# knowles-group/iterative-solver

Measured on AMD Instinct MI355X. Metric: subspace-update GB/s (gemm_inner+axpy) at N=1e8, 8 roots; 1/2/4/8 GPU, higher is better.
Workload: dtype f64

## Files before the change

iterative-solver_amd/csrc/context.hip:

```cpp
#include <immintrin.h>

#include <unistd.h>

#include <algorithm>
#include <atomic>
#include <chrono>
#include <condition_variable>
#include <cstdio>
#include <cstdlib>
#include <cstring>
#include <memory>
#include <mutex>
#include <thread>

#include "ssp_internal.h"

namespace {
thread_local std::string g_last_error;

size_t round_block(size_t bytes) {
  if (bytes < (size_t(1) << 20)) return (bytes + 255) & ~size_t(255);
  const size_t g = size_t(2) << 20;
  return (bytes + g - 1) / g * g;
}
// ... 380 lines not shown

int ssp_ledger_entry(ssp_ctx* ctx, int i, const char** name, long long* calls, double* kernel_ms, double* bytes) {
  SSP_CHECK_CTX(ctx);
  SSP_TRY(ssp::ledger_resolve(ctx));
  if (i < 0 || size_t(i) >= ctx->ledger.size()) return ssp::set_error(SSP_ERR_ARG, "ssp_ledger_entry: bad index");
  const auto& e = ctx->ledger[i];
  if (name) *name = e.name.c_str();
  if (calls) *calls = e.calls;
  if (kernel_ms) *kernel_ms = e.ms;
  if (bytes) *bytes = e.bytes;
  return SSP_OK;
}

const char* ssp_last_error(void) { return g_last_error.c_str(); }

const char* ssp_version(void) { return "subspace_hip 0.1 (gfx950, fp64)"; }

int ssp_device_count(void) {
  int n = 0;
  if (hipGetDeviceCount(&n) != hipSuccess) return 0;
  return n;
}

int ssp_ctx_create(int device, ssp_ctx** out) {
  if (!out) return ssp::set_error(SSP_ERR_ARG, "ssp_ctx_create: null out");
  *out = nullptr;
  int ndev = 0;
  SSP_TRY_HIP(hipGetDeviceCount(&ndev));
  if (device < 0 || device >= ndev)
    return ssp::set_error(SSP_ERR_ARG, "ssp_ctx_create: device " + std::to_string(device) + " not present");
  SSP_TRY_HIP(hipSetDevice(device));
  auto* ctx = new ssp_ctx();
  ctx->device = device;
  hipDeviceProp_t prop;
  if (hipGetDeviceProperties(&prop, device) == hipSuccess && prop.multiProcessorCount > 0)
    ctx->num_cus = prop.multiProcessorCount;
  if (const char* rs = std::getenv("SSP_ROW_SHAPE")) ctx->row_stride = std::string(rs) == "stride";
  if (const char* pc = std::getenv("SSP_PUBLISH")) ctx->publish_copy = std::string(pc) == "copy";
  if (const char* ex = std::getenv("SSP_EXACT_MAX")) ctx->exact_max = size_t(std::strtoull(ex, nullptr, 10));
  if (const char* ip = std::getenv("SSP_INNER_PER_CU")) ctx->inner_per_cu = std::max(1, std::atoi(ip));
  if (const char* op = std::getenv("SSP_OUTER_WG_PER_CU")) ctx->outer_per_cu = std::max(1, std::atoi(op));
  if (const char* fp = std::getenv("SSP_FUSED_PER_CU")) ctx->fused_per_cu = std::max(1, std::atoi(fp));
  if (const char* tw = std::getenv("SSP_TRANSFORM_WIDE")) ctx->transform_wide = std::atoi(tw) != 0;
  if (const char* sm = std::getenv("SSP_SELECT_MERGE")) ctx->select_rank = std::string(sm) != "tree";
  if (const char* lt = std::getenv("SSP_LEDGER_TIMING")) ctx->ledger_dispatch = std::string(lt) == "dispatch";
  ctx->ledger_detail = std::getenv("SSP_LEDGER_DETAIL") != nullptr;
  if (const char* ss = std::getenv("SSP_SYNTH_SHAPE")) {
    ctx->synth_stride = std::string(ss) == "stride";
    ctx->synth_window = std::string(ss) == "window";
  }
  if (const char* sm = std::getenv("SSP_SYNTH_MERGE")) ctx->synth_merge = std::atoi(sm) != 0;
  if (const char* df = std::getenv("SSP_DEFER_FILL")) ctx->defer_fill = std::atoi(df) != 0;
  if (const char* dout = std::getenv("SSP_DEFER_OUTER")) ctx->defer_outer = std::atoi(dout) != 0;
  if (const char* ct = std::getenv("SSP_COMM_TIMEOUT_S")) {
    const double v = std::atof(ct);
    if (v > 0) ctx->comm_timeout_s = v;
  }
  if (hipStreamCreateWithFlags(&ctx->stream, hipStreamNonBlocking) != hipSuccess) {
    delete ctx;
    return ssp::set_error(SSP_ERR_HIP, "hipStreamCreate failed");
  }
  int s = ssp::ensure_partial(ctx, size_t(1) << 20);
  if (s == SSP_OK) s = ssp::ensure_result(ctx, size_t(1) << 16);
  if (s == SSP_OK) {
    const size_t bytes = sizeof(unsigned) * ssp::kFoldLine * (ssp::kFoldShards + 1);
    if (hipMalloc(reinterpret_cast<void**>(&ctx->fold_counter), bytes) != hipSuccess ||
        hipMemsetAsync(ctx->fold_counter, 0, bytes, ctx->stream) != hipSuccess)
      s = ssp::set_error(SSP_ERR_NOMEM, "allocation of the reduction counter failed");
  }
  if (s != SSP_OK) {
    ssp_ctx_destroy(ctx);
    return s;
  }
  *out = ctx;
  return SSP_OK;
}

int ssp_ctx_destroy(ssp_ctx* ctx) {
  if (!ctx) return SSP_OK;
  (void)hipSetDevice(ctx->device);
  ctx->pending_fills.clear();
  ctx->pending_outer.discard();
  (void)ssp::p2p_detach(ctx);
  if (ctx->stream) (void)hipStreamSynchronize(ctx->stream);
  if (ctx->comm) ncclCommDestroy(ctx->comm);
  if (ctx->dev_err_host) (void)hipHostFree(ctx->dev_err_host);
  for (auto& e : ctx->ledger)
    for (auto& pr : e.pending) {
      (void)hipEventDestroy(pr.first);
      (void)hipEventDestroy(pr.second);
    }
  for (auto ev : ctx->event_pool) (void)hipEventDestroy(ev);
  for (auto& b : ctx->free_blocks) (void)hipFree(b.second);
  for (auto& b : ctx->live_blocks) (void)hipFree(b.first);
  if (ctx->partial) (void)hipFree(ctx->partial);
  if (ctx->result_dev) (void)hipFree(ctx->result_dev);
  if (ctx->result_host) (void)hipHostFree(ctx->result_host);
  if (ctx->pub_flag) (void)hipHostFree(ctx->pub_flag);
  if (ctx->fold_counter) (void)hipFree(ctx->fold_counter);
  if (ctx->async_dev) (void)hipFree(ctx->async_dev);
  if (ctx->async_host) (void)hipHostFree(ctx->async_host);
  if (ctx->async_flag) (void)hipHostFree(ctx->async_flag);
  if (ctx->synth_mask) (void)hipFree(ctx->synth_mask);
  if (ctx->ring_dev) (void)hipFree(ctx->ring_dev);
  if (ctx->ring_host) (void)hipHostFree(ctx->ring_host);
  for (auto& r : ctx->retired_rings) {
    if (r.first) (void)hipFree(r.first);
    if (r.second) (void)hipHostFree(r.second);
  }
  if (ctx->stream) (void)hipStreamDestroy(ctx->stream);
  delete ctx;
  return SSP_OK;
}

void* ssp_ctx_stream(ssp_ctx* ctx) {
  if (!ctx) return nullptr;
  (void)ssp::enter(ctx);
  return reinterpret_cast<void*>(ctx->stream);
}

int ssp_synchronize(ssp_ctx* ctx) {
  SSP_CHECK_CTX(ctx);
  return ssp::sync_stream(ctx, "synchronize");
}

int ssp_alloc(ssp_ctx* ctx, size_t n, double** out) {
  SSP_CHECK_CTX(ctx);
  if (!out) return ssp::set_error(SSP_ERR_ARG, "ssp_alloc: null out");
  const size_t bytes = round_block(std::max<size_t>(n, 1) * sizeof(double));
  auto it = ctx->free_blocks.find(bytes);
  void* p = nullptr;
  if (it != ctx->free_blocks.end()) {
    p = it->second;
    ctx->free_blocks.erase(it);
    ctx->bytes_cached -= bytes;
  } else {
    hipError_t e = hipMalloc(&p, bytes);
    if (e != hipSuccess) {
      (void)hipGetLastError();
      (void)hipStreamSynchronize(ctx->stream);
      for (auto& b : ctx->free_blocks) (void)hipFree(b.second);
      ctx->free_blocks.clear();
      ctx->bytes_cached = 0;
      if (hipMalloc(&p, bytes) != hipSuccess) {
        (void)hipGetLastError();
        return ssp::set_error(SSP_ERR_NOMEM, "ssp_alloc: out of HBM for " + std::to_string(bytes) + " bytes");
      }
    }
// ... 208 lines not shown
```

iterative-solver_amd/csrc/kernels_panel.hip:

```cpp
#include <algorithm>
#include <cstdio>
#include <cstddef>
#include <cstdlib>
#include <vector>

#include "ssp_internal.h"

namespace {

using ssp::kBlock;

__device__ __forceinline__ double2 ld2(const double* p) { return *reinterpret_cast<const double2*>(p); }
template <bool SC>
__device__ __forceinline__ double2 sc2(double2 v, double s) {
  return SC ? make_double2(v.x * s, v.y * s) : v;
}
template <bool SC>
__device__ __forceinline__ double sc1(double v, double s) {
  return SC ? v * s : v;
}

struct InnerArgs {
  const double* x[ssp::kInnerRows];
  const double* y[ssp::kInnerCols];
// ... 222 lines not shown
        }
#pragma unroll
        for (int j = 0; j < K; ++j)
#pragma unroll
          for (int u = 0; u < U; ++u) {
            acc[j][u & 1] = fma(xv[u].x, yv[j][u].x, acc[j][u & 1]);
            acc[j][u & 1] = fma(xv[u].y, yv[j][u].y, acc[j][u & 1]);
          }
      },
      [&](size_t p) {
        const double2 xv = sc2<SC>(ld2(a.x[0] + 2 * p), xs);
#pragma unroll
        for (int j = 0; j < K; ++j) {
          const double2 yv = sc2<SC>(ld2(a.y[j] + 2 * p), ys[j]);
          acc[j][0] = fma(xv.x, yv.x, acc[j][0]);
          acc[j][0] = fma(xv.y, yv.y, acc[j][0]);
        }
      },
      [&](size_t e) {
#pragma unroll
        for (int j = 0; j < K; ++j) acc[j][0] = fma(sc1<SC>(a.x[0][e], xs), sc1<SC>(a.y[j][e], ys[j]), acc[j][0]);
      });
  __shared__ double red[kBlock / 64][K];
  const int lane = threadIdx.x & 63, wave = threadIdx.x >> 6;
#pragma unroll
  for (int j = 0; j < K; ++j) {
    double v = acc[j][0] + acc[j][1];
#pragma unroll
    for (int off = 32; off > 0; off >>= 1) v += __shfl_down(v, off, 64);
    if (lane == 0) red[wave][j] = v;
  }
  __syncthreads();
  if (int(threadIdx.x) < K) {
    double v = red[0][threadIdx.x];
#pragma unroll
    for (int w = 1; w < kBlock / 64; ++w) v += red[w][threadIdx.x];
    ssp::store_partial(a.partial + size_t(blockIdx.x) * K + threadIdx.x, v);
  }
  if (a.tail.counter) ssp::fold_tail<K>(a.partial, a.tail);
}

struct OuterArgs {
  const double* x[ssp::kOuterSrc];
  double* y[ssp::kOuterDst];
  int k;
  int m;
  int set;
  int epi_mask;
  size_t n;
  const double* alpha_dev;
  const double* scale_dev;
  double alpha[ssp::kOuterAlpha];
  double epi[ssp::kOuterDst];
};
static_assert(sizeof(OuterArgs) <= 4000, "kernel argument block too large");
static_assert(ssp::PendingOuter::kSrc == ssp::kOuterSrc && ssp::PendingOuter::kDst == ssp::kOuterDst,
              "pending_outer.h records one launch");

constexpr int kOuterWin = 4;

template <int M, bool DEV, bool SET, bool SC = false, bool EPI = false>
__global__ __launch_bounds__(kBlock) void k_gemm_outer(const OuterArgs a) {
  static_assert(!EPI || (SET && !SC), "the epilogue rides on the unscaled write-only form");
  using ssp::ld2nt;
  using ssp::st2nt;
  using cdouble = const __attribute__((address_space(4))) double;
  const auto alpha = [&](int idx) { return DEV ? ((cdouble*)a.alpha_dev)[idx] : a.alpha[idx]; };
  const auto scale = [&](int idx) { return SC ? ((cdouble*)a.scale_dev)[idx] : 1.0; };
  constexpr int U = M > 8 ? 2 : kOuterWin;
  const int lane = threadIdx.x & 63;
  const size_t gw = size_t(blockIdx.x) * (kBlock / 64) + (threadIdx.x >> 6);
  const size_t nw = size_t(gridDim.x) * (kBlock / 64);
  const size_t n2 = a.n >> 1, win = 64 * U;
  const double2 z2 = make_double2(0, 0);
  for (size_t c = gw; c * win < n2; c += nw) {
    const size_t p0 = c * win + lane;
    bool ok[U];
#pragma unroll
    for (int u = 0; u < U; ++u) ok[u] = p0 + 64 * u < n2;
    double2 acc[U][M];
#pragma unroll
    for (int u = 0; u < U; ++u)
#pragma unroll
      for (int j = 0; j < M; ++j) acc[u][j] = (j < a.m && ok[u] && !SET) ? ld2nt(a.y[j] + 2 * (p0 + 64 * u)) : z2;
    if constexpr (SC && !SET) {
#pragma unroll
      for (int u = 0; u < U; ++u)
#pragma unroll
        for (int j = 0; j < M; ++j)
          if (j < a.m) acc[u][j] = sc2<SC>(acc[u][j], scale(a.k + j));
    }
    int i = 0;
    for (; i + 4 <= a.k; i += 4) {
      double2 xv[4][U];
#pragma unroll
      for (int b = 0; b < 4; ++b)
#pragma unroll
        for (int u = 0; u < U; ++u) xv[b][u] = ok[u] ? ld2nt(a.x[i + b] + 2 * (p0 + 64 * u)) : z2;
      if constexpr (SC) {
#pragma unroll
        for (int b = 0; b < 4; ++b)
#pragma unroll
          for (int u = 0; u < U; ++u) xv[b][u] = sc2<SC>(xv[b][u], scale(i + b));
      }
#pragma unroll
      for (int b = 0; b < 4; ++b)
#pragma unroll
        for (int j = 0; j < M; ++j) {
          if (j < a.m) {
            const double al = alpha((i + b) * a.m + j);
#pragma unroll
            for (int u = 0; u < U; ++u) {
              acc[u][j].x = fma(al, xv[b][u].x, acc[u][j].x);
              acc[u][j].y = fma(al, xv[b][u].y, acc[u][j].y);
            }
          }
        }
    }
    for (; i < a.k; ++i) {
      double2 xv[U];
#pragma unroll
      for (int u = 0; u < U; ++u) xv[u] = ok[u] ? ld2nt(a.x[i] + 2 * (p0 + 64 * u)) : z2;
      if constexpr (SC) {
#pragma unroll
        for (int u = 0; u < U; ++u) xv[u] = sc2<SC>(xv[u], scale(i));
      }
#pragma unroll
      for (int j = 0; j < M; ++j) {
        if (j < a.m) {
          const double al = alpha(i * a.m + j);
#pragma unroll
          for (int u = 0; u < U; ++u) {
            acc[u][j].x = fma(al, xv[u].x, acc[u][j].x);
            acc[u][j].y = fma(al, xv[u].y, acc[u][j].y);
          }
        }
      }
    }
    if constexpr (EPI) {
      constexpr int B = M == 8 ? 2 : 1;
#pragma unroll
      for (int j0 = 0; j0 < M; j0 += B) {
        double2 ev[B][U];
        bool on[B];
#pragma unroll
        for (int b = 0; b < B; ++b) {
          on[b] = j0 + b < a.m && ((a.epi_mask >> (j0 + b)) & 1);
          if (on[b]) {
#pragma unroll
            for (int u = 0; u < U; ++u) ev[b][u] = ok[u] ? ld2nt(a.x[a.k + j0 + b] + 2 * (p0 + 64 * u)) : z2;
          }
        }
#pragma unroll
        for (int b = 0; b < B; ++b) {
          if (on[b]) {
            const double ea = a.epi[j0 + b];
#pragma unroll
            for (int u = 0; u < U; ++u) {
              acc[u][j0 + b].x = fma(ea, ev[b][u].x, acc[u][j0 + b].x);
              acc[u][j0 + b].y = fma(ea, ev[b][u].y, acc[u][j0 + b].y);
            }
          }
        }
      }
    }
#pragma unroll
    for (int u = 0; u < U; ++u)
      if (ok[u])
#pragma unroll
        for (int j = 0; j < M; ++j)
          if (j < a.m) st2nt(a.y[j] + 2 * (p0 + 64 * u), acc[u][j]);
  }
  if ((a.n & 1) && blockIdx.x == 0 && threadIdx.x < a.m) {
    const size_t e = a.n - 1;
    const int j = threadIdx.x;
    double v = SET ? 0.0 : sc1<SC>(a.y[j][e], scale(a.k + j));
    for (int i = 0; i < a.k; ++i) v = fma(alpha(i * a.m + j), sc1<SC>(a.x[i][e], scale(i)), v);
    if constexpr (EPI) {
      if ((a.epi_mask >> j) & 1) v = fma(a.epi[j], a.x[a.k + j][e], v);
    }
    a.y[j][e] = v;
  }
}

struct AxpyInnerArgs {
  const double* x;
  const double* z;
  double* y[ssp::kOuterDst];
  double c[ssp::kOuterDst];
  int m;
  size_t n;
  double* partial;
  ssp::FoldTail tail;
};

constexpr int kFusedU = 4;

template <int M>
__global__ __launch_bounds__(kBlock) void k_axpy_inner(const AxpyInnerArgs a) {
  using ssp::ld2nt;
  using ssp::st2nt;
  double acc[M];
#pragma unroll
  for (int j = 0; j < M; ++j) acc[j] = 0;
  ssp::for_windows<kFusedU>(
      a.n,
      [&](size_t p0) {
        double2 xv[kFusedU], zv[kFusedU];
#pragma unroll
        for (int u = 0; u < kFusedU; ++u) xv[u] = ld2nt(a.x + 2 * (p0 + 64 * u));
#pragma unroll
        for (int u = 0; u < kFusedU; ++u) zv[u] = ld2nt(a.z + 2 * (p0 + 64 * u));
#pragma unroll
        for (int j = 0; j < M; ++j) {
          if (j < a.m) {
            double2 y[kFusedU];
#pragma unroll
            for (int u = 0; u < kFusedU; ++u) y[u] = ld2nt(a.y[j] + 2 * (p0 + 64 * u));
#pragma unroll
            for (int u = 0; u < kFusedU; ++u) {
              y[u].x = fma(a.c[j], xv[u].x, y[u].x);
              y[u].y = fma(a.c[j], xv[u].y, y[u].y);
              st2nt(a.y[j] + 2 * (p0 + 64 * u), y[u]);
              acc[j] = fma(y[u].x, zv[u].x, acc[j]);
// ... 672 lines not shown
template <bool SC>
int launch_inner_sym_t(ssp_ctx* ctx, const InnerArgs& a, unsigned grid) {
  switch ((a.m + 3) / 4) {
    case 1: launch_inner_sym_g<1, SC>(ctx, a, grid); break;
    case 2: launch_inner_sym_g<2, SC>(ctx, a, grid); break;
    case 3: launch_inner_sym_g<3, SC>(ctx, a, grid); break;
    default: launch_inner_sym_g<4, SC>(ctx, a, grid); break;
  }
  SSP_TRY_HIP(hipGetLastError());
  return SSP_OK;
}

int launch_inner_sym(ssp_ctx* ctx, const InnerArgs& a, unsigned grid, bool sc) {
  return sc ? launch_inner_sym_t<true>(ctx, a, grid) : launch_inner_sym_t<false>(ctx, a, grid);
}

template <bool SC>
int launch_inner_sc(ssp_ctx* ctx, const InnerArgs& a, unsigned grid, bool pre) {
  const int mg = (a.m + 3) / 4, need = (a.k + 3) / 4;
  switch (mg) {
    case 1: return launch_inner_mg<1, SC>(ctx, grid, a, need, pre);
    case 2: return launch_inner_mg<2, SC>(ctx, grid, a, need, pre);
    case 3: return launch_inner_mg<3, SC>(ctx, grid, a, need, false);
    default: return launch_inner_mg<4, SC>(ctx, grid, a, need, false);
  }
}

int launch_inner(ssp_ctx* ctx, const InnerArgs& a, unsigned grid, bool sc, bool pre = false) {
  return sc ? launch_inner_sc<true>(ctx, a, grid, pre) : launch_inner_sc<false>(ctx, a, grid, pre);
}

template <bool DEV, bool SET, bool SC, bool EPI = false>
void launch_outer_t(ssp_ctx* ctx, unsigned grid, const OuterArgs& a) {
  if (a.m <= 1)
    SSP_LAUNCH((k_gemm_outer<1, DEV, SET, SC, EPI>), dim3(grid), dim3(kBlock), 0, ctx->stream, a);
  else if (a.m <= 2)
    SSP_LAUNCH((k_gemm_outer<2, DEV, SET, SC, EPI>), dim3(grid), dim3(kBlock), 0, ctx->stream, a);
  else if (a.m <= 4)
    SSP_LAUNCH((k_gemm_outer<4, DEV, SET, SC, EPI>), dim3(grid), dim3(kBlock), 0, ctx->stream, a);
  else if (a.m <= 8)
    SSP_LAUNCH((k_gemm_outer<8, DEV, SET, SC, EPI>), dim3(grid), dim3(kBlock), 0, ctx->stream, a);
  else
    SSP_LAUNCH((k_gemm_outer<16, DEV, SET, SC, EPI>), dim3(grid), dim3(kBlock), 0, ctx->stream, a);
}

template <bool SC>
void launch_outer_sc(ssp_ctx* ctx, unsigned grid, const OuterArgs& a) {
  if (a.alpha_dev)
    a.set ? launch_outer_t<true, true, SC>(ctx, grid, a) : launch_outer_t<true, false, SC>(ctx, grid, a);
  else
    a.set ? launch_outer_t<false, true, SC>(ctx, grid, a) : launch_outer_t<false, false, SC>(ctx, grid, a);
}

int launch_outer(ssp_ctx* ctx, const OuterArgs& a) {
  const unsigned grid = ssp::stream_grid(ctx, a.n / 2 + 1, kOuterWin, unsigned(ctx->outer_per_cu));
  if (a.epi_mask) {
    if (!a.set || a.scale_dev || a.k + a.m > ssp::kOuterSrc)
      return ssp::set_error(SSP_ERR_ARG, "gemm_outer: epilogue terms on a launch that cannot carry them");
    a.alpha_dev ? launch_outer_t<true, true, false, true>(ctx, grid, a)
                : launch_outer_t<false, true, false, true>(ctx, grid, a);
    SSP_TRY_HIP(hipGetLastError());
    return SSP_OK;
  }
  a.scale_dev ? launch_outer_sc<true>(ctx, grid, a) : launch_outer_sc<false>(ctx, grid, a);
  SSP_TRY_HIP(hipGetLastError());
  return SSP_OK;
}

int ng_inst(int need) { return need <= 4 ? need : need <= 6 ? 6 : need <= 8 ? 8 : need <= 12 ? 12 : 16; }
std::string shape_tag(const char* kind, int a, int b, int c, int d, bool sc) {
  char t[96];
  std::snprintf(t, sizeof(t), "%s<%d,%d> %dx%d%s", kind, a, b, c, d, sc ? " sc" : "");
  return t;
}

bool any_scaled(const double* s, int n) {
  for (int i = 0; s && i < n; ++i)
    if (s[i] != 1.0) return true;
  return false;
}

}

extern "C" {

int ssp_gemm_inner(ssp_ctx* ctx, const double* const* xx, int m, const double* const* yy, int k, size_t n,
                   double* out) {
  return ssp_gemm_inner_scaled(ctx, xx, nullptr, m, yy, nullptr, k, n, out);
}

int ssp_gemm_inner_scaled(ssp_ctx* ctx, const double* const* xx, const double* xs, int m, const double* const* yy,
                          const double* ys, int k, size_t n, double* out) {
  SSP_CHECK_CTX(ctx);
  if (m < 0 || k < 0) return ssp::set_error(SSP_ERR_ARG, "ssp_gemm_inner: negative dimension");
  if (m * k > 0 && !out) return ssp::set_error(SSP_ERR_ARG, "ssp_gemm_inner: null out");
  if (m == 0 || k == 0) return SSP_OK;
  SSP_TRY(check_ptrs(xx, m, n, "ssp_gemm_inner"));
  SSP_TRY(check_ptrs(yy, k, n, "ssp_gemm_inner"));
  const bool swap = m > k;
  const double* const* rows = swap ? yy : xx;
  const double* const* cols = swap ? xx : yy;
  const int R = swap ? k : m, C = swap ? m : k;
  std::vector<double> rs(size_t(R), 1.0), cs(size_t(C), 1.0);
  for (int i = 0; i < m; ++i) (swap ? cs : rs)[size_t(i)] = xs ? xs[i] : 1.0;
  for (int j = 0; j < k; ++j) (swap ? rs : cs)[size_t(j)] = ys ? ys[j] : 1.0;
  const bool sc = any_scaled(rs.data(), R) || any_scaled(cs.data(), C);
  int pad = -1;
// ... 85 lines not shown
        const int cols_per_launch = 4 * ng_max((mr + 3) / 4);
        for (int c0 = 0; c0 < C2; c0 += cols_per_launch) {
          InnerArgs a{};
          a.m = mr;
          a.k = std::min(cols_per_launch, C2 - c0);
          a.n = n;
          for (int i = 0; i < a.m; ++i) {
            a.x[i] = rows[r0 + i];
            a.xs[i] = rs[size_t(r0 + i)];
          }
          for (int j = 0; j < a.k; ++j) {
            a.y[j] = cols[c0 + j];
            a.ys[j] = cs[size_t(c0 + j)];
          }
          const bool sc_launch = any_scaled(a.xs, a.m) || any_scaled(a.ys, a.k);
          const unsigned grid = inner_grid(ctx, n);
          SSP_TRY(ssp::ensure_partial(ctx, size_t(grid) * a.m * a.k));
          a.partial = ctx->partial;
          const bool pre = pad >= 0 && c0 == 0;
          if (r0 == 0 && c0 == 0)
            ls.detail(shape_tag(pre ? "mfma-pre" : "mfma", (a.m + 3) / 4, ng_inst((a.k + 3) / 4), a.m, a.k, sc_launch));
          SSP_TRY(launch_inner(ctx, a, grid, sc_launch, pre));
          const bool last = r0 + ssp::kInnerRows >= R && c0 + cols_per_launch >= C2;
          SSP_TRY(ssp::launch_reduce_partials(ctx, ctx->partial, int(grid), a.m, a.k, ctx->result_dev, C2, r0, c0, &tail,
                                              last));
        }
      }
    }
  }
  std::vector<double> t(swap || pad >= 0 ? total : 0);
  double* dst = swap || pad >= 0 ? t.data() : out;
  if (tail.counter) {
    SSP_TRY(ssp::fold_finish(ctx, tail, dst));
  } else {
    SSP_TRY(ssp::reduce_fetch(ctx, dst, total));
  }
  if (pad >= 0) {
    for (int i = 0; i < R; ++i)
      for (int j = 0; j < C; ++j) t[size_t(i) * C + j] = t[size_t(i) * C2 + (j < R ? j : j + pad)];
    if (!swap) {
      std::copy(t.begin(), t.begin() + long(size_t(R) * C), out);
      return SSP_OK;
    }
  }
  if (!swap) return SSP_OK;
  for (int i = 0; i < m; ++i)
    for (int j = 0; j < k; ++j) out[size_t(i) * k + j] = t[size_t(j) * m + i];
  return SSP_OK;
}

}

namespace {
int launch_record(ssp_ctx* ctx, const ssp::PendingOuter::Record& r) {
  const int e = r.terms();
  ssp::LedgerScope ls(ctx, r.set ? "gemm_outer_set" : "gemm_outer", 8.0 * r.n * (r.k + r.m + e));
  OuterArgs a{};
  a.k = r.k;
  a.m = r.m;
  a.set = 1;
  a.n = r.n;
  for (int i = 0; i < r.k; ++i) a.x[i] = r.x[i];
  for (int j = 0; j < r.m; ++j) a.y[j] = r.y[j];
  if (e > 0) {
    a.epi_mask = int(r.mask);
    for (int j = 0; j < r.m; ++j) {
      const bool on = (r.mask >> j) & 1u;
      a.x[r.k + j] = on ? r.ex[j] : nullptr;
      a.epi[j] = on ? r.ea[j] : 0.0;
    }
  }
  const bool dev = r.k * r.m > ssp::kOuterAlpha;
  if (dev) {
    void* p;
    SSP_TRY(ssp::upload_small(ctx, r.alpha, size_t(r.k) * r.m * sizeof(double), &p));
    a.alpha_dev = static_cast<const double*>(p);
    SSP_TRY(ssp::flush_uploads(ctx));
  } else {
    std::copy(r.alpha, r.alpha + r.k * r.m, a.alpha);
  }
  const int mi = a.m <= 1 ? 1 : a.m <= 2 ? 2 : a.m <= 4 ? 4 : a.m <= 8 ? 8 : 16;
  std::string tag = shape_tag(dev ? "dev" : "arg", mi, a.set, a.k, a.m, false);
  if (e > 0) tag += " epi" + std::to_string(e);
  ls.detail(tag);
  return launch_outer(ctx, a);
}
}

namespace ssp {
int flush_outer(ssp_ctx* ctx) {
  if (!ctx->pending_outer.pending()) return SSP_OK;
  int status = SSP_OK;
  ctx->pending_outer.flush([&](const PendingOuter::Record& r) { status = launch_record(ctx, r); });
  return status;
}
}

namespace {
int gemm_outer_impl(ssp_ctx* ctx, const double* alphas, const double* const* xx, const double* xs, int k,
                    double* const* yy, const double* ys, int m, size_t n, bool set) {
  SSP_CHECK_CTX_KEEP_FILLS(ctx);
  if (m < 0 || k < 0) return ssp::set_error(SSP_ERR_ARG, "ssp_gemm_outer: negative dimension");
  if (set && k == 0) {
    for (int j = 0; j < m; ++j) SSP_TRY(ssp_fill(ctx, 0.0, yy[j], n));
    return SSP_OK;
  }
  if (m == 0 || n == 0) return SSP_OK;
  if (k == 0) {
    for (int j = 0; j < m; ++j)
      if (!set && ys && ys[j] != 1.0) SSP_TRY(ssp_scal(ctx, ys[j], yy[j], n));
    return SSP_OK;
  }
  if (!alphas) return ssp::set_error(SSP_ERR_ARG, "ssp_gemm_outer: null alphas");
  SSP_TRY(check_ptrs(xx, k, n, "ssp_gemm_outer"));
  SSP_TRY(check_ptrs(const_cast<const double* const*>(yy), m, n, "ssp_gemm_outer"));
  for (int j = 0; j < m; ++j)
    for (int i = 0; i < k; ++i)
      if (yy[j] == xx[i]) return ssp::set_error(SSP_ERR_ARG, "ssp_gemm_outer: a destination aliases a source");
  bool consume = false;
  if (!ctx->pending_fills.empty()) {
    for (int i = 0; i < k; ++i) SSP_TRY(ssp::flush_fills_over(ctx, xx[i], n));
    if (set) {
      for (int j = 0; j < m; ++j) SSP_TRY(ssp::overwrite_fills(ctx, yy[j], n));
    } else {
      consume = !any_scaled(ys, m) && !ssp::exact_mode(ctx, n);
      for (int j = 0; consume && j < m; ++j) {
        consume = ctx->pending_fills.find_exact(yy[j], n) >= 0;
        for (int i = 0; consume && i < j; ++i) consume = yy[i] != yy[j];
      }
      for (int j = 0; j < m; ++j) {
        if (consume) ctx->pending_fills.erase(ctx->pending_fills.find_exact(yy[j], n));
        else SSP_TRY(ssp::flush_fills_over(ctx, yy[j], n));
      }
    }
  }
  const bool set0 = set || consume;
  if (ctx->defer_outer && set0 && !any_scaled(xs, k) && !ssp::exact_mode(ctx, n) &&
      ctx->pending_outer.record(alphas, xx, k, yy, m, n, set))
    return SSP_OK;
  ssp::LedgerScope ls(ctx, set ? "gemm_outer_set" : "gemm_outer", 8.0 * n * (k + (set0 ? 1.0 : 2.0) * m));
  if (ssp::exact_mode(ctx, n)) return ssp::exact_outer(ctx, alphas, xx, xs, k, yy, ys, m, n, set);
  for (int j0 = 0; j0 < m; j0 += ssp::kOuterDst) {
    const int mm = std::min(ssp::kOuterDst, m - j0);
    for (int i0 = 0; i0 < k; i0 += ssp::kOuterSrc) {
      OuterArgs a{};
      a.m = mm;
// ... 448 lines not shown
```

iterative-solver_amd/csrc/kernels_stream.hip:

```cpp
#include <algorithm>
#include <cmath>

#include "ssp_internal.h"

namespace {

using ssp::kBlock;

__device__ __forceinline__ double2 ld2(const double* p) { return *reinterpret_cast<const double2*>(p); }
__device__ __forceinline__ void st2(double* p, double2 v) { *reinterpret_cast<double2*>(p) = v; }
template <bool SC>
__device__ __forceinline__ double2 sc2(double2 v, double s) {
  return SC ? make_double2(v.x * s, v.y * s) : v;
}
template <bool SC>
__device__ __forceinline__ double sc1(double v, double s) {
  return SC ? v * s : v;
}

using ssp::kWinMin;
using ssp::kWinU;
constexpr int kDotU = 4;


__device__ __forceinline__ double block_sum(double v) {
  __shared__ double wsum[kBlock / 64];
#pragma unroll
  for (int off = 32; off > 0; off >>= 1) v += __shfl_down(v, off, 64);
  const int lane = threadIdx.x & 63, wave = threadIdx.x >> 6;
  if (lane == 0) wsum[wave] = v;
  __syncthreads();
  double s = 0;
  if (threadIdx.x == 0) {
#pragma unroll
    for (int w = 0; w < kBlock / 64; ++w) s += wsum[w];
  }
  return s;
}

__global__ __launch_bounds__(kBlock) void k_fill(double* __restrict__ x, size_t n, double alpha) {
  const size_t n2 = n >> 1;
  const size_t stride = size_t(gridDim.x) * kBlock;
  const double2 v = make_double2(alpha, alpha);
  for (size_t i = size_t(blockIdx.x) * kBlock + threadIdx.x; i < n2; i += stride) st2(x + 2 * i, v);
  if ((n & 1) && blockIdx.x == 0 && threadIdx.x == 0) x[n - 1] = alpha;
}

__global__ __launch_bounds__(kBlock) void k_scal(double* __restrict__ x, size_t n, double alpha) {
  using ssp::ld2nt;
  using ssp::st2nt;
  const size_t n2 = n >> 1;
  const size_t stride = size_t(gridDim.x) * kBlock;
  size_t i = size_t(blockIdx.x) * kBlock + threadIdx.x;
  for (; i + 3 * stride < n2; i += 4 * stride) {
    double2 a0 = ld2nt(x + 2 * i), a1 = ld2nt(x + 2 * (i + stride)), a2 = ld2nt(x + 2 * (i + 2 * stride)),
            a3 = ld2nt(x + 2 * (i + 3 * stride));
    st2nt(x + 2 * i, make_double2(a0.x * alpha, a0.y * alpha));
    st2nt(x + 2 * (i + stride), make_double2(a1.x * alpha, a1.y * alpha));
    st2nt(x + 2 * (i + 2 * stride), make_double2(a2.x * alpha, a2.y * alpha));
    st2nt(x + 2 * (i + 3 * stride), make_double2(a3.x * alpha, a3.y * alpha));
  }
  for (; i < n2; i += stride) {
    double2 a = ld2(x + 2 * i);
    st2(x + 2 * i, make_double2(a.x * alpha, a.y * alpha));
  }
  if ((n & 1) && blockIdx.x == 0 && threadIdx.x == 0) x[n - 1] *= alpha;
}

template <bool SC>
__global__ __launch_bounds__(kBlock) void k_copy(double* __restrict__ x, const double* __restrict__ y, size_t n,
                                                 double alpha) {
  using ssp::ld2nt;
  using ssp::st2nt;
  const size_t n2 = n >> 1;
  const size_t stride = size_t(gridDim.x) * kBlock;
// ... 290 lines not shown
int ssp_fill(ssp_ctx* ctx, double alpha, double* x, size_t n) {
  SSP_CHECK_CTX_KEEP_FILLS(ctx);
  if (ctx->defer_fill && n > 0 && alpha == 0.0 && !std::signbit(alpha) && !ssp::exact_mode(ctx, n)) {
    SSP_TRY(check_vec(x, n, "ssp_fill"));
    ssp::FillFlusher f{ctx};
    ctx->pending_fills.insert(x, n, f);
    return f.status;
  }
  SSP_TRY(ssp::overwrite_fills(ctx, x, n));
  return ssp::fill_now(ctx, alpha, x, n);
}

int ssp_scal(ssp_ctx* ctx, double alpha, double* x, size_t n) {
  SSP_CHECK_CTX(ctx);
  SSP_TRY(check_vec(x, n, "ssp_scal"));
  if (n == 0) return SSP_OK;
  ssp::LedgerScope ls(ctx, "scal", 16.0 * n);
  if (n >= kWinMin)
    SSP_LAUNCH(k_scal_win, dim3(ssp::win_grid(ctx, n, kWinU, 16)), dim3(kBlock), 0, ctx->stream, x, n, alpha);
  else
    SSP_LAUNCH(k_scal, dim3(ssp::stream_grid(ctx, n / 2 + 1, 4, 64)), dim3(kBlock), 0, ctx->stream, x, n, alpha);
  SSP_TRY_HIP(hipGetLastError());
  return SSP_OK;
}

}

namespace {
int copy_impl(ssp_ctx* ctx, double alpha, double* x, const double* y, size_t n, bool scaled, const char* what) {
  SSP_CHECK_CTX_KEEP_FILLS(ctx);
  SSP_TRY(check_vec(x, n, what));
  SSP_TRY(check_vec(y, n, what));
  if (n == 0 || (x == y && !scaled)) return SSP_OK;
  if (x == y) return ssp_scal(ctx, alpha, x, n);
  SSP_TRY(ssp::flush_fills_over(ctx, y, n));
  SSP_TRY(ssp::overwrite_fills(ctx, x, n));
  ssp::LedgerScope ls(ctx, scaled ? "scal_copy" : "copy", 16.0 * n);
  if (n >= kWinMin) {
    const dim3 g(ssp::win_grid(ctx, n, kWinU, 16));
    if (scaled) SSP_LAUNCH(k_copy_win<true>, g, dim3(kBlock), 0, ctx->stream, x, y, n, alpha);
    else SSP_LAUNCH(k_copy_win<false>, g, dim3(kBlock), 0, ctx->stream, x, y, n, alpha);
  } else {
    const dim3 g(ssp::stream_grid(ctx, n / 2 + 1, 4, 64));
    if (scaled) SSP_LAUNCH(k_copy<true>, g, dim3(kBlock), 0, ctx->stream, x, y, n, alpha);
    else SSP_LAUNCH(k_copy<false>, g, dim3(kBlock), 0, ctx->stream, x, y, n, alpha);
  }
  SSP_TRY_HIP(hipGetLastError());
  return SSP_OK;
}

int axpy_impl(ssp_ctx* ctx, double alpha, const double* x, double xs, double* y, double ys, size_t n,
              const char* what) {
  SSP_CHECK_CTX_KEEP_ALL(ctx);
  const bool sc = xs != 1.0 || ys != 1.0;
  if (ctx->pending_outer.pending()) {
    const bool valid = n > 0 && x && y && ssp::aligned16(x) && ssp::aligned16(y);
    if (valid && !sc && ctx->pending_outer.attach(alpha, x, y, n)) return ssp::flush_fills_over(ctx, x, n);
    SSP_TRY(ssp::flush_outer(ctx));
  }
  SSP_TRY(ssp::flush_fills(ctx));
  SSP_TRY(check_vec(x, n, what));
  SSP_TRY(check_vec(y, n, what));
  if (n == 0) return SSP_OK;
  ssp::LedgerScope ls(ctx, "axpy", 24.0 * n);
  if (ssp::exact_mode(ctx, n)) return ssp::exact_outer(ctx, &alpha, &x, &xs, 1, &y, &ys, 1, n, false);
  if (n >= kWinMin) {
    const dim3 g(ssp::win_grid(ctx, n, kWinU, 16));
    if (sc) SSP_LAUNCH(k_axpy_win<true>, g, dim3(kBlock), 0, ctx->stream, x, y, n, alpha, xs, ys);
    else SSP_LAUNCH(k_axpy_win<false>, g, dim3(kBlock), 0, ctx->stream, x, y, n, alpha, xs, ys);
  } else {
    const dim3 g(ssp::stream_grid(ctx, n / 2 + 1, 4, 64));
    if (sc) SSP_LAUNCH(k_axpy<true>, g, dim3(kBlock), 0, ctx->stream, x, y, n, alpha, xs, ys);
    else SSP_LAUNCH(k_axpy<false>, g, dim3(kBlock), 0, ctx->stream, x, y, n, alpha, xs, ys);
  }
  SSP_TRY_HIP(hipGetLastError());
  return SSP_OK;
}

int dot_impl(ssp_ctx* ctx, const double* x, double xs, const double* y, double ys, size_t n, double* out,
             const char* what) {
  SSP_CHECK_CTX(ctx);
  if (!out) return ssp::set_error(SSP_ERR_ARG, std::string(what) + ": null out");
  SSP_TRY(check_vec(x, n, what));
  SSP_TRY(check_vec(y, n, what));
  if (n == 0) {
    SSP_TRY(ssp::ensure_result(ctx, 1));
    SSP_TRY_HIP(hipMemsetAsync(ctx->result_dev, 0, sizeof(double), ctx->stream));
    return ssp::reduce_fetch(ctx, out, 1);
  }
  if (ssp::exact_mode(ctx, n)) {
    ssp::FoldTail tail{};
    SSP_TRY(ssp::fold_begin(ctx, 1, &tail));
    {
      ssp::LedgerScope ls(ctx, "dot", (x == y && xs == ys ? 8.0 : 16.0) * n);
      SSP_TRY(ssp::exact_inner(ctx, &x, &xs, 1, &y, &ys, 1, n, false, tail));
    }
    return ssp::fold_finish(ctx, tail, out);
  }
  const unsigned grid = ssp::win_grid(ctx, n, kDotU, 8);
  SSP_TRY(ssp::ensure_partial(ctx, grid));
  ssp::FoldTail tail{};
  SSP_TRY(ssp::fold_begin(ctx, 1, &tail));
  {
    const bool same = x == y && xs == ys, sc = xs != 1.0 || ys != 1.0;
    ssp::LedgerScope ls(ctx, "dot", (same ? 8.0 : 16.0) * n);
    const dim3 g(grid);
    double* part = ctx->partial;
    if (same && sc) SSP_LAUNCH((k_dot_partial<true, true>), g, dim3(kBlock), 0, ctx->stream, x, y, n, part, tail, xs, ys);
    else if (same) SSP_LAUNCH((k_dot_partial<true, false>), g, dim3(kBlock), 0, ctx->stream, x, y, n, part, tail, xs, ys);
    else if (sc) SSP_LAUNCH((k_dot_partial<false, true>), g, dim3(kBlock), 0, ctx->stream, x, y, n, part, tail, xs, ys);
    else SSP_LAUNCH((k_dot_partial<false, false>), g, dim3(kBlock), 0, ctx->stream, x, y, n, part, tail, xs, ys);
    SSP_TRY_HIP(hipGetLastError());
  }
  return ssp::fold_finish(ctx, tail, out);
}
}

extern "C" {

int ssp_copy(ssp_ctx* ctx, double* x, const double* y, size_t n) { return copy_impl(ctx, 1.0, x, y, n, false, "ssp_copy"); }

int ssp_scal_copy(ssp_ctx* ctx, double alpha, double* x, const double* y, size_t n) {
  return copy_impl(ctx, alpha, x, y, n, true, "ssp_scal_copy");
}

int ssp_axpy(ssp_ctx* ctx, double alpha, const double* x, double* y, size_t n) {
  return axpy_impl(ctx, alpha, x, 1.0, y, 1.0, n, "ssp_axpy");
}

int ssp_axpy_scaled(ssp_ctx* ctx, double alpha, const double* x, double xs, double* y, double ys, size_t n) {
  return axpy_impl(ctx, alpha, x, xs, y, ys, n, "ssp_axpy_scaled");
}

int ssp_dot(ssp_ctx* ctx, const double* x, const double* y, size_t n, double* out) {
// ... 31 lines not shown
```

iterative-solver_amd/csrc/ssp_internal.h:

```cpp
#pragma once
#include <hip/hip_ext.h>
#include <hip/hip_runtime.h>
#include <rccl/rccl.h>

#include <cstddef>
#include <cstdint>
#include <map>
#include <string>
#include <unordered_map>
#include <vector>

#include "pending_fill.h"
#include "pending_outer.h"
#include "subspace_hip.h"

struct ssp_ledger_entry_t {
  std::string name;
  long long calls = 0;
  double ms = 0;
  double bytes = 0;
  std::vector<std::pair<hipEvent_t, hipEvent_t>> pending;
};

namespace ssp {
struct P2PComm;
}

struct ssp_ctx {
  int device = 0;
  bool ledger_on = false;
  std::vector<ssp_ledger_entry_t> ledger;
  std::vector<hipEvent_t> event_pool;
  int num_cus = 256;
  int inner_per_cu = 4;
  int outer_per_cu = 8;
  int fused_per_cu = 8;
  bool select_rank = true;
  bool transform_wide = true;
  bool synth_stride = false;
  bool ledger_dispatch = false;
  bool ledger_detail = false;
  bool synth_window = false;
  bool synth_merge = true;
  bool row_stride = false;
  bool publish_copy = false;
  bool defer_fill = true;
  ssp::PendingFills pending_fills;
  bool defer_outer = true;
  ssp::PendingOuter pending_outer;
  hipStream_t stream = nullptr;

  std::multimap<size_t, void*> free_blocks;
  std::unordered_map<void*, size_t> live_blocks;
  size_t bytes_in_use = 0;
  size_t bytes_cached = 0;

  double* partial = nullptr;
  size_t partial_cap = 0;
  double* result_dev = nullptr;
  double* result_host = nullptr;
  size_t result_cap = 0;
  unsigned long long* pub_flag = nullptr;
  unsigned long long pub_seq = 0;
  unsigned* fold_counter = nullptr;
  double* async_dev = nullptr;
  double* async_host = nullptr;
  unsigned long long* async_flag = nullptr;
  unsigned long long async_seq = 0;
  bool async_pending = false;
  bool async_launched = false;
  size_t async_n = 0;
  std::vector<double> async_sync;

  char* ring_host = nullptr;
  char* ring_dev = nullptr;
  size_t ring_cap = 0;
  size_t ring_head = 0;
  size_t ring_pending = 0;
  std::vector<std::pair<char*, char*>> retired_rings;

  unsigned short* synth_mask = nullptr;
  size_t synth_mask_n = 0, synth_mask_offset = 0;
  unsigned long long synth_mask_seed = 0;
  int synth_mask_rank = 0;

  ncclComm_t comm = nullptr;
  ssp_host_allreduce_fn host_allreduce = nullptr;
  ssp_host_allgather_fn host_allgather = nullptr;
  void* host_user = nullptr;
  ssp::P2PComm* p2p = nullptr;
  int nranks = 1;
  int rank = 0;
  double comm_timeout_s = 300.0;
  size_t exact_max = 2048;
  bool comm_failed = false;
  std::string comm_fail_msg;
  int* dev_err_host = nullptr;
};

namespace ssp {

constexpr int kBlock = 256;
constexpr int kInnerRows = 16;
constexpr int kInnerCols = 64;
constexpr int kOuterSrc = 64;
constexpr int kOuterDst = 16;
constexpr int kOuterAlpha = 384;
constexpr int kPrecVec = 16;
constexpr int kSelectTile = 2048;
constexpr int kWinU = 8;
constexpr size_t kWinMin = size_t(1) << 24;

int set_error(int code, const std::string& msg);
int hip_error(hipError_t e, const char* what);
int use_device(ssp_ctx* ctx);
int fill_now(ssp_ctx* ctx, double alpha, double* x, size_t n);
int flush_fills(ssp_ctx* ctx);
int flush_fills_over(ssp_ctx* ctx, const void* p, size_t n);
int overwrite_fills(ssp_ctx* ctx, const void* p, size_t n);
int flush_outer(ssp_ctx* ctx);
int enter(ssp_ctx* ctx);
int ensure_partial(ssp_ctx* ctx, size_t n_doubles);
int ensure_result(ssp_ctx* ctx, size_t n_doubles);
int upload_small(ssp_ctx* ctx, const void* host, size_t bytes, void** dev);
int flush_uploads(ssp_ctx* ctx);
int allreduce_dev(ssp_ctx* ctx, double* buf, size_t n);
int agree_exact_max(ssp_ctx* ctx);
int rccl_settle(ssp_ctx* ctx, ncclResult_t r, const char* what);
int fetch_result(ssp_ctx* ctx, double* out, size_t n);
int reduce_fetch(ssp_ctx* ctx, double* out, size_t n);
int wait_flag(ssp_ctx* ctx, unsigned long long seq, bool* seen, const char* what = "reduction",
              const unsigned long long* flag = nullptr);
constexpr size_t kAsyncResults = 64 * 32;
int ensure_async(ssp_ctx* ctx);
unsigned stream_grid(const ssp_ctx* ctx, size_t work_items, unsigned per_thread, unsigned blocks_per_cu = 8);

typedef double nt_double2 __attribute__((ext_vector_type(2)));
__device__ __forceinline__ double2 ld2nt(const double* p) {
  const nt_double2 v = __builtin_nontemporal_load(reinterpret_cast<const nt_double2*>(p));
  return make_double2(v.x, v.y);
}
__device__ __forceinline__ void st2nt(double* p, double2 v) {
  const nt_double2 w = {v.x, v.y};
  __builtin_nontemporal_store(w, reinterpret_cast<nt_double2*>(p));
}
bool aligned16(const void* p);

class LedgerScope {
 public:
  LedgerScope(ssp_ctx* ctx, const char* op, double bytes);
  ~LedgerScope();
  LedgerScope(const LedgerScope&) = delete;
  LedgerScope& operator=(const LedgerScope&) = delete;
  void detail(const std::string& tag);
  static bool dispatch_events(hipStream_t stream, hipEvent_t* start, hipEvent_t* stop);

 private:
  ssp_ctx* ctx_;
  int slot_ = -1;
  hipEvent_t start_ = nullptr;
  hipEvent_t stop_ = nullptr;
  bool launched_ = false;
  double last_bytes_ = 0;
  LedgerScope* prev_ = nullptr;
};

#define SSP_LAUNCH(K, G, B, SHM, ST, ...)                                                  \
  do {                                                                                    \
    hipEvent_t ssp_e0_ = nullptr, ssp_e1_ = nullptr;                                      \
    if (::ssp::LedgerScope::dispatch_events(ST, &ssp_e0_, &ssp_e1_))                      \
      hipExtLaunchKernelGGL(K, G, B, SHM, ST, ssp_e0_, ssp_e1_, 0u, __VA_ARGS__);         \
    else                                                                                  \
      hipLaunchKernelGGL(K, G, B, SHM, ST, __VA_ARGS__);                                  \
// ... 211 lines not shown
```

Baseline: 7008.

## Fuse squared norms of deferred gemm_outer outputs into the outer kernel

When a self-dot is requested on a vector that a pending deferred gemm_outer will write, the outer launch now runs a norm-carrying variant. That variant accumulates per-output sums of squares in shared memory and folds them through the partial/fold-tail reduction path. The norms are cached so later self-dots on those outputs return without rereading the vectors, which saves a full pass over memory for each norm. The cost is extra shared memory and register pressure in the outer kernel, a different grid shape, and cache-invalidation logic that must stay correct across axpy and flush calls.

```diff
diff --git a/iterative-solver_amd/csrc/context.hip b/iterative-solver_amd/csrc/context.hip
--- a/iterative-solver_amd/csrc/context.hip
+++ b/iterative-solver_amd/csrc/context.hip
@@ -456,6 +456,7 @@
   if (const char* sm = std::getenv("SSP_SYNTH_MERGE")) ctx->synth_merge = std::atoi(sm) != 0;
   if (const char* df = std::getenv("SSP_DEFER_FILL")) ctx->defer_fill = std::atoi(df) != 0;
   if (const char* dout = std::getenv("SSP_DEFER_OUTER")) ctx->defer_outer = std::atoi(dout) != 0;
+  if (const char* on = std::getenv("SSP_OUTER_NORMS")) ctx->outer_norms_on = std::atoi(on) != 0;
   if (const char* ct = std::getenv("SSP_COMM_TIMEOUT_S")) {
     const double v = std::atof(ct);
     if (v > 0) ctx->comm_timeout_s = v;
@@ -498,6 +499,7 @@
   for (auto& b : ctx->free_blocks) (void)hipFree(b.second);
   for (auto& b : ctx->live_blocks) (void)hipFree(b.first);
   if (ctx->partial) (void)hipFree(ctx->partial);
+  if (ctx->norms_dev) (void)hipFree(ctx->norms_dev);
   if (ctx->result_dev) (void)hipFree(ctx->result_dev);
   if (ctx->result_host) (void)hipHostFree(ctx->result_host);
   if (ctx->pub_flag) (void)hipHostFree(ctx->pub_flag);
diff --git a/iterative-solver_amd/csrc/kernels_panel.hip b/iterative-solver_amd/csrc/kernels_panel.hip
--- a/iterative-solver_amd/csrc/kernels_panel.hip
+++ b/iterative-solver_amd/csrc/kernels_panel.hip
@@ -298,16 +298,26 @@
   const double* scale_dev;
   double alpha[ssp::kOuterAlpha];
   double epi[ssp::kOuterDst];
+  double* partial;
+  ssp::FoldTail tail;
 };
 static_assert(sizeof(OuterArgs) <= 4000, "kernel argument block too large");
 static_assert(ssp::PendingOuter::kSrc == ssp::kOuterSrc && ssp::PendingOuter::kDst == ssp::kOuterDst,
               "pending_outer.h records one launch");
 
 constexpr int kOuterWin = 4;
-
-template <int M, bool DEV, bool SET, bool SC = false, bool EPI = false>
+static_assert(kOuterWin == ssp::kDotU, "the norm-carrying instance walks k_dot_partial's windows");
+
+template <int M>
+__device__ __forceinline__ double* outer_norm_acc() {
+  __shared__ double acc[M * kOuterWin * kBlock];
+  return acc;
+}
+
+template <int M, bool DEV, bool SET, bool SC = false, bool EPI = false, bool NRM = false>
 __global__ __launch_bounds__(kBlock) void k_gemm_outer(const OuterArgs a) {
   static_assert(!EPI || (SET && !SC), "the epilogue rides on the unscaled write-only form");
+  static_assert(!NRM || (SET && !SC && M <= 8), "the norms ride on the unscaled write-only form, 4-position windows");
   using ssp::ld2nt;
   using ssp::st2nt;
   using cdouble = const __attribute__((address_space(4))) double;
@@ -319,11 +329,17 @@
   const size_t nw = size_t(gridDim.x) * (kBlock / 64);
   const size_t n2 = a.n >> 1, win = 64 * U;
   const double2 z2 = make_double2(0, 0);
-  for (size_t c = gw; c * win < n2; c += nw) {
+  double* nacc = nullptr;
+  if constexpr (NRM) {
+    nacc = outer_norm_acc<M>() + threadIdx.x;
+#pragma unroll
+    for (int q = 0; q < M * U; ++q) nacc[q * kBlock] = 0;
+  }
+  for (size_t c = gw; NRM ? c < n2 / win : c * win < n2; c += nw) {
     const size_t p0 = c * win + lane;
     bool ok[U];
 #pragma unroll
-    for (int u = 0; u < U; ++u) ok[u] = p0 + 64 * u < n2;
+    for (int u = 0; u < U; ++u) ok[u] = NRM || p0 + 64 * u < n2;
     double2 acc[U][M];
 #pragma unroll
     for (int u = 0; u < U; ++u)
@@ -416,6 +432,80 @@
 #pragma unroll
         for (int j = 0; j < M; ++j)
           if (j < a.m) st2nt(a.y[j] + 2 * (p0 + 64 * u), acc[u][j]);
+    if constexpr (NRM) {
+#pragma unroll
+      for (int j = 0; j < M; ++j)
+        if (j < a.m) {
+#pragma unroll
+          for (int u = 0; u < U; ++u) {
+            double s = nacc[(j * U + u) * kBlock];
+            s = fma(acc[u][j].x, acc[u][j].x, s);
+            s = fma(acc[u][j].y, acc[u][j].y, s);
+            nacc[(j * U + u) * kBlock] = s;
+          }
+          __builtin_amdgcn_sched_barrier(0);
+        }
+    }
+  }
+  if constexpr (NRM) {
+    if (blockIdx.x == 0) {
+      const size_t p = (n2 / win) * win + threadIdx.x;
+      if (p < n2) {
+        for (int j = 0; j < a.m; ++j) {
+          double2 v = z2;
+          for (int i = 0; i < a.k; ++i) {
+            const double al = alpha(i * a.m + j);
+            const double2 xv = ld2(a.x[i] + 2 * p);
+            v.x = fma(al, xv.x, v.x);
+            v.y = fma(al, xv.y, v.y);
+          }
+          if constexpr (EPI) {
+            if ((a.epi_mask >> j) & 1) {
+              const double2 ev = ld2(a.x[a.k + j] + 2 * p);
+              v.x = fma(a.epi[j], ev.x, v.x);
+              v.y = fma(a.epi[j], ev.y, v.y);
+            }
+          }
+          *reinterpret_cast<double2*>(a.y[j] + 2 * p) = v;
+          double s = nacc[j * U * kBlock];
+          s = fma(v.x, v.x, s);
+          s = fma(v.y, v.y, s);
+          nacc[j * U * kBlock] = s;
+        }
+      }
+      if ((a.n & 1) && threadIdx.x == 0) {
+        const size_t e = a.n - 1;
+        for (int j = 0; j < a.m; ++j) {
+          double v = 0.0;
+          for (int i = 0; i < a.k; ++i) v = fma(alpha(i * a.m + j), a.x[i][e], v);
+          if constexpr (EPI) {
+            if ((a.epi_mask >> j) & 1) v = fma(a.epi[j], a.x[a.k + j][e], v);
+          }
+          a.y[j][e] = v;
+          nacc[j * U * kBlock] = fma(v, v, nacc[j * U * kBlock]);
+        }
+      }
+    }
+    __shared__ double red[kBlock / 64][M];
+#pragma unroll
+    for (int j = 0; j < M; ++j)
+      if (j < a.m) {
+        const double s0 = nacc[(j * U + 0) * kBlock], s1 = nacc[(j * U + 1) * kBlock];
+        const double s2 = nacc[(j * U + 2) * kBlock], s3 = nacc[(j * U + 3) * kBlock];
+        double v = (s0 + s1) + (s2 + s3);
+#pragma unroll
+        for (int off = 32; off > 0; off >>= 1) v += __shfl_down(v, off, 64);
+        if (lane == 0) red[threadIdx.x >> 6][j] = v;
+      }
+    __syncthreads();
+    if (int(threadIdx.x) < a.m) {
+      double s = 0;
+#pragma unroll
+      for (int w = 0; w < kBlock / 64; ++w) s += red[w][threadIdx.x];
+      ssp::store_partial(a.partial + size_t(blockIdx.x) * a.m + threadIdx.x, s);
+    }
+    ssp::fold_tail<M>(a.partial, a.tail);
+    return;
   }
   if ((a.n & 1) && blockIdx.x == 0 && threadIdx.x < a.m) {
     const size_t e = a.n - 1;
@@ -1194,7 +1284,33 @@
     a.set ? launch_outer_t<false, true, SC>(ctx, grid, a) : launch_outer_t<false, false, SC>(ctx, grid, a);
 }
 
+constexpr int kOuterNormDst = 8;
+unsigned outer_norm_grid(const ssp_ctx* ctx, size_t n) { return ssp::win_grid(ctx, n, ssp::kDotU, 8); }
+
+template <bool DEV, bool EPI>
+void launch_outer_nrm(ssp_ctx* ctx, unsigned grid, const OuterArgs& a) {
+  if (a.m <= 1)
+    SSP_LAUNCH((k_gemm_outer<1, DEV, true, false, EPI, true>), dim3(grid), dim3(kBlock), 0, ctx->stream, a);
+  else if (a.m <= 2)
+    SSP_LAUNCH((k_gemm_outer<2, DEV, true, false, EPI, true>), dim3(grid), dim3(kBlock), 0, ctx->stream, a);
+  else if (a.m <= 4)
+    SSP_LAUNCH((k_gemm_outer<4, DEV, true, false, EPI, true>), dim3(grid), dim3(kBlock), 0, ctx->stream, a);
+  else
+    SSP_LAUNCH((k_gemm_outer<8, DEV, true, false, EPI, true>), dim3(grid), dim3(kBlock), 0, ctx->stream, a);
+}
+
 int launch_outer(ssp_ctx* ctx, const OuterArgs& a) {
+  if (a.partial) {
+    if (!a.set || a.scale_dev || a.m > kOuterNormDst || (a.epi_mask && a.k + a.m > ssp::kOuterSrc))
+      return ssp::set_error(SSP_ERR_ARG, "gemm_outer: norms on a launch that cannot carry them");
+    const unsigned grid = outer_norm_grid(ctx, a.n);
+    if (a.epi_mask)
+      a.alpha_dev ? launch_outer_nrm<true, true>(ctx, grid, a) : launch_outer_nrm<false, true>(ctx, grid, a);
+    else
+      a.alpha_dev ? launch_outer_nrm<true, false>(ctx, grid, a) : launch_outer_nrm<false, false>(ctx, grid, a);
+    SSP_TRY_HIP(hipGetLastError());
+    return SSP_OK;
+  }
   const unsigned grid = ssp::stream_grid(ctx, a.n / 2 + 1, kOuterWin, unsigned(ctx->outer_per_cu));
   if (a.epi_mask) {
     if (!a.set || a.scale_dev || a.k + a.m > ssp::kOuterSrc)
@@ -1386,7 +1502,7 @@
 }
 
 namespace {
-int launch_record(ssp_ctx* ctx, const ssp::PendingOuter::Record& r) {
+int launch_record(ssp_ctx* ctx, const ssp::PendingOuter::Record& r, const ssp::FoldTail* norms = nullptr) {
   const int e = r.terms();
   ssp::LedgerScope ls(ctx, r.set ? "gemm_outer_set" : "gemm_outer", 8.0 * r.n * (r.k + r.m + e));
   OuterArgs a{};
@@ -1416,6 +1532,11 @@
   const int mi = a.m <= 1 ? 1 : a.m <= 2 ? 2 : a.m <= 4 ? 4 : a.m <= 8 ? 8 : 16;
   std::string tag = shape_tag(dev ? "dev" : "arg", mi, a.set, a.k, a.m, false);
   if (e > 0) tag += " epi" + std::to_string(e);
+  if (norms) {
+    a.partial = ctx->partial;
+    a.tail = *norms;
+    tag += " nrm";
+  }
   ls.detail(tag);
   return launch_outer(ctx, a);
 }
@@ -1423,9 +1544,48 @@
 
 namespace ssp {
 int flush_outer(ssp_ctx* ctx) {
+  ctx->outer_norms.forget();
   if (!ctx->pending_outer.pending()) return SSP_OK;
   int status = SSP_OK;
   ctx->pending_outer.flush([&](const PendingOuter::Record& r) { status = launch_record(ctx, r); });
+  return status;
+}
+
+bool outer_norms_apply(const ssp_ctx* ctx, const double* y, size_t n) {
+  if (!ctx->outer_norms_on || !ctx->pending_outer.pending()) return false;
+  const PendingOuter::Record& r = ctx->pending_outer.record();
+  if (r.m > kOuterNormDst || n != r.n) return false;
+  for (int j = 0; j < r.m; ++j)
+    if (r.y[j] == y) return true;
+  return false;
+}
+
+int launch_outer_norms(ssp_ctx* ctx) {
+  ctx->outer_norms.forget();
+  if (!ctx->pending_outer.pending()) return SSP_OK;
+  const PendingOuter::Record& r = ctx->pending_outer.record();
+  const int m = r.m;
+  const bool ranks = comm_attached(ctx);
+  FoldTail tail{};
+  int status = ensure_partial(ctx, size_t(outer_norm_grid(ctx, r.n)) * m);
+  if (status == SSP_OK) status = fold_begin(ctx, m, &tail);
+  if (status == SSP_OK && ranks) {
+    if (!ctx->norms_dev && hipMalloc(reinterpret_cast<void**>(&ctx->norms_dev), kOuterDst * sizeof(double)) != hipSuccess)
+      status = set_error(SSP_ERR_NOMEM, "hipMalloc of the norm staging failed");
+    tail.out = ctx->norms_dev;
+  }
+  if (status != SSP_OK) {
+    const int plain = flush_outer(ctx);
+    return plain != SSP_OK ? plain : status;
+  }
+  ctx->outer_norms.keep(r.y, m, r.n);
+  ctx->pending_outer.flush([&](const PendingOuter::Record& rec) { status = launch_record(ctx, rec, &tail); });
+  if (status == SSP_OK && !ranks) {
+    double v[kOuterDst];
+    status = fold_finish(ctx, tail, v);
+    if (status == SSP_OK) ctx->outer_norms.set_values(v);
+  }
+  if (status != SSP_OK) ctx->outer_norms.forget();
   return status;
 }
 }
diff --git a/iterative-solver_amd/csrc/kernels_stream.hip b/iterative-solver_amd/csrc/kernels_stream.hip
--- a/iterative-solver_amd/csrc/kernels_stream.hip
+++ b/iterative-solver_amd/csrc/kernels_stream.hip
@@ -20,7 +20,7 @@
 
 using ssp::kWinMin;
 using ssp::kWinU;
-constexpr int kDotU = 4;
+using ssp::kDotU;
 
 
 __device__ __forceinline__ double block_sum(double v) {
@@ -417,6 +417,7 @@
 int axpy_impl(ssp_ctx* ctx, double alpha, const double* x, double xs, double* y, double ys, size_t n,
               const char* what) {
   SSP_CHECK_CTX_KEEP_ALL(ctx);
+  ctx->outer_norms.forget();
   const bool sc = xs != 1.0 || ys != 1.0;
   if (ctx->pending_outer.pending()) {
     const bool valid = n > 0 && x && y && ssp::aligned16(x) && ssp::aligned16(y);
@@ -444,7 +445,23 @@
 
 int dot_impl(ssp_ctx* ctx, const double* x, double xs, const double* y, double ys, size_t n, double* out,
              const char* what) {
-  SSP_CHECK_CTX(ctx);
+  SSP_CHECK_CTX_KEEP_ALL(ctx);
+  if (out && x == y && xs == 1.0 && ys == 1.0) {
+    if (ssp::outer_norms_apply(ctx, y, n)) SSP_TRY(ssp::launch_outer_norms(ctx));
+    const int j = ctx->outer_norms.find(y, n);
+    if (j >= 0) {
+      if (!ssp::comm_attached(ctx)) {
+        *out = ctx->outer_norms.value(j);
+        return SSP_OK;
+      }
+      SSP_TRY(ssp::comm_check(ctx));
+      SSP_TRY(ssp::ensure_result(ctx, 1));
+      SSP_TRY_HIP(hipMemcpyAsync(ctx->result_dev, ctx->norms_dev + j, sizeof(double), hipMemcpyDeviceToDevice, ctx->stream));
+      return ssp::reduce_fetch(ctx, out, 1);
+    }
+  }
+  SSP_TRY(ssp::flush_outer(ctx));
+  SSP_TRY(ssp::flush_fills(ctx));
   if (!out) return ssp::set_error(SSP_ERR_ARG, std::string(what) + ": null out");
   SSP_TRY(check_vec(x, n, what));
   SSP_TRY(check_vec(y, n, what));
diff --git a/iterative-solver_amd/csrc/outer_norms.h b/iterative-solver_amd/csrc/outer_norms.h
--- /dev/null
+++ b/iterative-solver_amd/csrc/outer_norms.h
@@ -0,0 +1,48 @@
+#pragma once
+#include <cstddef>
+
+namespace ssp {
+
+class OuterNorms {
+ public:
+  static constexpr int kDst = 16;
+
+  bool empty() const { return m_ == 0; }
+  int size() const { return m_; }
+
+  bool keep(double* const* y, int m, size_t n) {
+    forget();
+    if (m < 1 || m > kDst || n == 0) return false;
+    for (int j = 0; j < m; ++j) {
+      y_[j] = y[j];
+      v_[j] = 0.0;
+    }
+    n_ = n;
+    m_ = m;
+    return true;
+  }
+  void set_values(const double* v) {
+    for (int j = 0; j < m_; ++j) v_[j] = v[j];
+  }
+
+  int find(const double* y, size_t n) const {
+    if (n != n_) return -1;
+    for (int j = 0; j < m_; ++j)
+      if (y_[j] == y) return j;
+    return -1;
+  }
+  double value(int j) const { return v_[j]; }
+
+  void forget() {
+    m_ = 0;
+    n_ = 0;
+  }
+
+ private:
+  const double* y_[kDst] = {};
+  double v_[kDst] = {};
+  size_t n_ = 0;
+  int m_ = 0;
+};
+
+}
diff --git a/iterative-solver_amd/csrc/ssp_internal.h b/iterative-solver_amd/csrc/ssp_internal.h
--- a/iterative-solver_amd/csrc/ssp_internal.h
+++ b/iterative-solver_amd/csrc/ssp_internal.h
@@ -12,6 +12,7 @@
 
 #include "pending_fill.h"
 #include "pending_outer.h"
+#include "outer_norms.h"
 #include "subspace_hip.h"
 
 struct ssp_ledger_entry_t {
@@ -48,6 +49,9 @@
   ssp::PendingFills pending_fills;
   bool defer_outer = true;
   ssp::PendingOuter pending_outer;
+  bool outer_norms_on = true;
+  ssp::OuterNorms outer_norms;
+  double* norms_dev = nullptr;
   hipStream_t stream = nullptr;
 
   std::multimap<size_t, void*> free_blocks;
@@ -110,6 +114,7 @@
 constexpr int kSelectTile = 2048;
 constexpr int kWinU = 8;
 constexpr size_t kWinMin = size_t(1) << 24;
+constexpr int kDotU = 4;
 
 int set_error(int code, const std::string& msg);
 int hip_error(hipError_t e, const char* what);
@@ -119,6 +124,8 @@
 int flush_fills_over(ssp_ctx* ctx, const void* p, size_t n);
 int overwrite_fills(ssp_ctx* ctx, const void* p, size_t n);
 int flush_outer(ssp_ctx* ctx);
+bool outer_norms_apply(const ssp_ctx* ctx, const double* y, size_t n);
+int launch_outer_norms(ssp_ctx* ctx);
 int enter(ssp_ctx* ctx);
 int ensure_partial(ssp_ctx* ctx, size_t n_doubles);
 int ensure_result(ssp_ctx* ctx, size_t n_doubles);
```

After: 7240 (median of 6 runs). 1.03x the previous value.
